# Audio-WestlakeU/FS-EEND

Measured on AMD Instinct MI355X. Metric: audio frames/sec (T=500 chunks), higher is better.
Workload: dtype bf16

## Files before the change

fs-eend_amd/build.py:

```python
import os
import subprocess
import sys
from concurrent.futures import ThreadPoolExecutor

HERE = os.path.dirname(os.path.abspath(__file__))
CSRC = os.path.join(HERE, "csrc")
SOURCES = ["gemm.hip", "ffn.hip", "ffn_stream.hip", "convert_f32.hip", "convert_rows.hip", "encin.hip", "conv_stream.hip", "proj.hip", "attn.hip", "attn_full.hip", "attn_stream.hip", "spk_stream.hip", "embloss.hip", "postproc.hip", "feature.hip", "pit.hip", "misc.hip", "retention.hip", "retention_full.hip", "ret_stream.hip", "stream.hip", "stream_multi.hip", "skinny.hip", "gemm_f32.hip", "api.hip",
           "wgrad.hip", "ffn_train_stream.hip", "proj_stream.hip", "gemm_acc_stream.hip", "attn_bwd.hip", "attn_bwd_fused.hip", "train_rows.hip", "embloss_bwd.hip", "optim.hip", "api_train.hip",
           "ls_train.hip", "retention_bwd.hip"]
LIB = os.path.join(CSRC, "libeend_hip.so")
ARCH = "gfx950"
FLAGS = ["-O3", "-std=c++17", "-fPIC", f"--offload-arch={ARCH}", "-fno-gpu-rdc"]


def _hipcc():
    for c in (os.environ.get("HIPCC"), "/opt/rocm/bin/hipcc", "hipcc"):
        if c and (os.path.isabs(c) and os.path.exists(c) or not os.path.isabs(c)):
            return c
    return "hipcc"


def _stale(target, deps):
    if not os.path.exists(target):
        return True
# ... 36 lines not shown
```

fs-eend_amd/csrc/api.hip:

```cpp
#include "../../include/eend_hip.h"
#include "kernels.h"
#include <stdlib.h>
#include <string.h>

namespace {
GemmParams base_params(const void* A, int lda, const void* W, int ldw, const float* bias, int M, int N, int K) {
    GemmParams p;
    memset(&p, 0, sizeof(p));
    p.A = A; p.lda = lda; p.W = W; p.ldw = ldw; p.bias = bias;
    p.M = M; p.N = N; p.K = K; p.ldo = N; p.Tp = 64; p.H = 4; p.dh = 64; p.C = 1;
    p.alpha = 1.0f; p.eps = 1e-5f; p.conv_cin = 64; p.conv_pad = 0; p.drop.scale = 1.0f;
#ifdef EEND_GEMM_ABLATE
    const char* d = getenv("EEND_GEMM_DBG");
    p.dbg = d ? atoi(d) : 0;
#endif
    return p;
}
}

extern "C" {

int eend_abi_version(void) { return 5; }

int eend_bn_cast_pad_f16(const float* x, const float* bn_weight, const float* bn_bias, const float* bn_mean,
// ... 240 lines not shown
    return eend_launch_conv_stream(p, (hipStream_t)stream);
}

int eend_encoder_input_ok(int Fin, int Tp, int ldw) { return eend_encin_supported(Fin, Tp, ldw); }

int eend_encoder_input_f16(const float* const* x_ptrs, const int* lens, float pad_value, const float* bn_w, const float* bn_b,
                           const float* bn_mean, const float* bn_var, float bn_eps, const void* W_f16, int ldw, const float* bias,
                           const float* gamma, const float* beta, float eps, float* out_f32, void* out_f16, int B, int T, int Tp,
                           int Fin, void* stream) {
    EncInParams p;
    memset(&p, 0, sizeof(p));
    p.x_ptrs = x_ptrs; p.lens = lens; p.pad_value = pad_value; p.bn_w = bn_w; p.bn_b = bn_b; p.bn_mean = bn_mean; p.bn_var = bn_var;
    p.bn_eps = bn_eps; p.W = W_f16; p.ldw = ldw; p.bias = bias; p.gamma = gamma; p.beta = beta; p.eps = eps; p.out32 = out_f32;
    p.out16 = out_f16; p.B = B; p.T = T; p.Tp = Tp; p.Fin = Fin;
    return eend_launch_encin(p, (hipStream_t)stream);
}

int eend_spk_stream_elems(void) { return (int)eend_spk_stream_nelems(); }

int eend_spk_stream_ok(int C, int Tp) { return eend_spk_stream_supported(C, Tp); }

int eend_spk_stream_pack_f16(const void* Wo, const void* W_in, void* stream_out, void* stream) {
    return eend_launch_spk_stream_pack(Wo, W_in, stream_out, (hipStream_t)stream);
}

int eend_attnout_spk_stream_f16(const void* A, int lda, const void* wstream, const float* bo, const void* res_f16,
                                const float* g1, const float* be1, float eps1, void* x_f16, const float* b_in, void* O_f16,
                                int B, int C, int Tp, float scale, void* stream) {
    SpkStreamParams p;
    memset(&p, 0, sizeof(p));
// ... 344 lines not shown
```

fs-eend_amd/csrc/kernels.h:

```cpp
#pragma once
#include <hip/hip_runtime.h>
#include <stdint.h>
#include "../../include/eend_hip.h"
#include "common.h"

enum GemmEpilogue {
    EPI_PLAIN_F16 = 0,
    EPI_PLAIN_RELU_F16 = 1,
    EPI_QK_HEADS = 2,
    EPI_VT_HEADS = 3,
    EPI_RES_LN = 4,
    EPI_L2NORM = 5,
    EPI_CONVERT = 6,
    EPI_RES_SCALE = 7,
    EPI_RES_SCALE_LN16 = 8,
    EPI_PLAIN_SWISH_F16 = 9,
    EPI_GLU_F16 = 10,
    EPI_QK_HEADS_F16 = 11,
    EPI_KTVT_HEADS_F16 = 12,
    EPI_PLAIN_BF16 = 13,
    EPI_MASK_BF16 = 14,
    EPI_F32_ROWMASK = 15,
    EPI_RES_LN_TRAIN = 16,
    EPI_L2NORM_TRAIN = 17,
// ... 267 lines not shown
    const float* be1;
    float eps1;
    const void* res16;
    void* x16;
    const float* res32;
    float* x32;
    const float* bin;
    void* O;
    int B, C, Tp;
    float scale;
};
long eend_spk_stream_nelems();
int eend_spk_stream_supported(int C, int Tp);
int eend_launch_spk_stream_pack(const void* Wo, const void* Win, void* out, hipStream_t stream);
int eend_launch_spk_stream(const SpkStreamParams& p, hipStream_t stream);
int eend_launch_convert_fanout_rows(const void* E, const void* W1, const float* pc, float* out32, void* out16, int B, int Tp, int C,
                                    hipStream_t stream);
struct ConvStreamParams {
    const void* X;
    const void* wstream;
    const float* bias;
    const int* ilens;
    float* out32;
    void* out16;
    float* inv_norm;
    int nseq, Tp, ktaps, pad;
};
long eend_conv_stream_nelems(int ktaps);
int eend_conv_stream_supported(int cin, int ktaps, int pad);
int eend_launch_conv_stream_pack(const void* Wr, void* out, int ktaps, hipStream_t stream);
// ... 191 lines not shown
```

fs-eend_amd/fs_model.py:

```python
import copy
import math
from typing import List, Optional, Sequence

import torch
import torch.nn as nn
from torch import Tensor

from . import ops
from .lib import EendHipError

_D_SUPPORTED = 256
_H_SUPPORTED = 4


class PositionalEncoding(nn.Module):

    def __init__(self, d_model, dropout=0.1, max_len=5000):
        super().__init__()
        self.dropout = nn.Dropout(p=dropout)
        pe = torch.zeros(max_len, d_model)
        position = torch.arange(0, max_len, dtype=torch.float).unsqueeze(1)
        div_term = torch.exp(torch.arange(0, d_model, 2).float() * (-math.log(10000.0) / d_model))
        pe[:, 0::2] = torch.sin(position * div_term)
        pe[:, 1::2] = torch.cos(position * div_term)
# ... 205 lines not shown
        dl = []
        for l in self.dec.attractor_decoder.layers:
            dl.append(dict(
                in1_w=_f16(_qscaled(l.self_attn1.in_proj_weight)), in1_b=_f32(_qscaled(l.self_attn1.in_proj_bias)),
                out1_w=_f16(l.self_attn1.out_proj.weight), out1_b=_f32(l.self_attn1.out_proj.bias),
                in2_w=_f16(l.self_attn2.in_proj_weight), in2_b=_f32(l.self_attn2.in_proj_bias),
                out2_w=_f16(l.self_attn2.out_proj.weight), out2_b=_f32(l.self_attn2.out_proj.bias),
                w1=_f16(l.linear1.weight), b1=_f32(l.linear1.bias), w2=_f16(l.linear2.weight), b2=_f32(l.linear2.bias),
                g11=_f32(l.norm11.weight), be11=_f32(l.norm11.bias), eps11=l.norm11.eps,
                g21=_f32(l.norm21.weight), be21=_f32(l.norm21.bias), eps21=l.norm21.eps,
                g22=_f32(l.norm22.weight), be22=_f32(l.norm22.bias), eps22=l.norm22.eps))
        for L in dl:
            if ops.stream_ok(L["w1"].shape[0]):
                L["ws"] = ops.ffn_stream_pack(L["out2_w"], L["w1"], L["w2"])
            L["ws1"] = ops.spk_stream_pack(L["out1_w"], L["in2_w"])
            L["in1_wp"] = ops.inproj_attn_pack(L["in1_w"])
        P["dec.layers"] = dl
        self._prep, self._prep_key = P, key
        self._pc = {}
        return P

    def _convert_const(self, C):
        if C not in self._pc:
            from . import lib as _lib
            D = self.enc.n_units if hasattr(self.enc, "n_units") else self.n_units
            dev = self.dec.convert.weight.device
            W = self.dec.convert.weight.detach().to(torch.float32).contiguous()
            b = self.dec.convert.bias.detach().to(torch.float32).contiguous()
            pe = self.dec.pos_enc.pe[0, :C].to(device=dev, dtype=torch.float32).contiguous()
            pc = torch.empty(C, D, dtype=torch.float32, device=dev)
# ... 66 lines not shown
                                       L["be2"], L["eps2"], None, ws.h16)
            else:
                ops.attnout_ffn_fused_res16(o16, L["out_w"], L["out_b"], ws.h16, L["g1"], L["be1"], L["eps1"], L["w1"], L["b1"],
                                            L["w2"], L["b2"], L["g2"], L["be2"], L["eps2"], None, ws.h16)

        emb32 = torch.empty(Me, D, dtype=torch.float32, device=dev)
        if "cnn.ws" in P:
            ops.conv1d_l2norm_stream(ws.h16, P["cnn.ws"], P["cnn.b"], il, emb32, ws.emb16, B, Tp, P["cnn.k"], P["cnn.pad"])
        else:
            ops.conv1d_l2norm(ws.h16, P["cnn.w"], P["cnn.b"], il, emb32, ws.emb16, B, Tp, D, P["cnn.k"], P["cnn.pad"])

        ops.convert_fanout(ws.emb16, P["convert.w1"], self._convert_const(C), None, ws.a16, B, Tp, C)
        o16 = ws.o16[:Md]
        for L in P["dec.layers"]:
            time_attention(ws.a16, L, "in1_w", "in1_b", B * C, self.dec.mask_delay, T)
            ops.attnout_spk_stream(o16, L["ws1"], L["out1_b"], ws.a16, L["g11"], L["be11"], L["eps11"], ws.a16, L["in2_b"], o16, B, C, Tp)
            if "ws" in L:
                ops.attnout_ffn_stream(o16, L["ws"], L["out2_b"], None, ws.a16, L["g21"], L["be21"], L["eps21"], L["b1"], L["b2"],
                                       L["g22"], L["be22"], L["eps22"], None, ws.a16)
            else:
                ops.attnout_ffn_fused_res16(o16, L["out2_w"], L["out2_b"], ws.a16, L["g21"], L["be21"], L["eps21"], L["w1"], L["b1"],
                                            L["w2"], L["b2"], L["g22"], L["be22"], L["eps22"], None, ws.a16)

        attr = torch.empty(B, T, C, D, dtype=torch.float32, device=dev)
        logits = torch.empty(B, T, C, dtype=torch.float32, device=dev)
        ops.head_l2dot(emb32, ws.a16, attr, logits, B, T, Tp, C, D)
        emb = emb32.view(B, Tp, D)
        return logits, emb, attr, T, Tp

    @torch.no_grad()
# ... 23 lines not shown
```

fs-eend_amd/lib.py:

```python
import ctypes
import os

_HERE = os.path.dirname(os.path.abspath(__file__))
LIB_PATH = os.environ.get("EEND_HIP_LIB") or os.path.join(_HERE, "csrc", "libeend_hip.so")

_vp, _i, _f = ctypes.c_void_p, ctypes.c_int, ctypes.c_float
_l = ctypes.c_long

ABI_VERSION = 5

PROTOTYPES = {
    "eend_abi_version": [],
    "eend_bn_cast_pad_f16": [_vp, _vp, _vp, _vp, _vp, _f, _vp, _i, _i, _i, _i, _i, _i, _vp],
    "eend_gather_bn_cast_pad_f16": [_vp, _vp, _f, _vp, _vp, _vp, _vp, _f, _vp, _i, _i, _i, _i, _i, _i, _vp],
    "eend_linear_f16": [_vp, _i, _vp, _i, _vp, _vp, _i, _i, _i, _i, _i, _vp],
    "eend_inproj_heads_bf16": [_vp, _i, _vp, _i, _vp, _vp, _vp, _vp, _i, _i, _i, _i, _i, _vp],
    "eend_linear_glu_f16": [_vp, _i, _vp, _i, _vp, _vp, _i, _i, _i, _i, _vp],
    "eend_linear_res_ln_f16": [_vp, _i, _vp, _i, _vp, _vp, _f, _vp, _vp, _f, _vp, _vp, _i, _i, _vp],
    "eend_linear_res16_ln_f16": [_vp, _i, _vp, _i, _vp, _vp, _f, _vp, _vp, _f, _vp, _vp, _i, _i, _vp],
    "eend_linear_res_scale_ln16_f16": [_vp, _i, _vp, _i, _vp, _vp, _f, _vp, _vp, _f, _vp, _vp, _i, _i, _vp],
    "eend_ffn_fused_f16": [_vp, _i, _vp, _vp, _vp, _vp, _vp, _f, _vp, _vp, _f, _vp, _vp, _i, _i, _i, _i, _vp],
    "eend_attnout_ffn_fused_f16": [_vp, _i, _vp, _vp, _vp, _vp, _vp, _f, _vp, _vp, _vp, _vp, _vp, _vp, _f, _vp, _vp, _vp, _vp, _i, _i, _vp],
    "eend_attnout_ffn_fused_res16_f16": [_vp, _i, _vp, _vp, _vp, _vp, _vp, _f, _vp, _vp, _vp, _vp, _vp, _vp, _f, _vp, _vp, _i, _i, _vp],
    "eend_convert_fanout_f32": [_vp, _vp, _i, _vp, _vp, _vp, _vp, _i, _i, _i, _vp],
# ... 15 lines not shown
    "eend_gemm_acc_stream_elems": [_i],
    "eend_gemm_acc_stream_ok": [_i, _i, _i],
    "eend_gemm_acc_stream_pack_bf16": [_vp, _i, _vp, _i, _vp],
    "eend_gemm_acc_stream_bf16": [_vp, _i, _vp, _vp, _i, _i, _vp],
    "eend_proj_stream_elems": [_i],
    "eend_proj_stream_pack_f16": [_vp, _vp, _i, _vp],
    "eend_proj_stream_ok": [_i, _i, _i, _i, _i, _vp],
    "eend_proj_stream_f16": [_vp, _i, _vp, _vp, _i, _i, _i, _i, _vp, _vp],
    "eend_inproj_attn_long_scratch_elems": [_i, _i, _i, _i, _vp, _vp],
    "eend_inproj_attn_causal_long_f16": [_vp, _i, _vp, _vp, _vp, _vp, _vp, _i, _i, _i, _i, _i, _i, _vp],
    "eend_spk_stream_elems": [],
    "eend_spk_stream_ok": [_i, _i],
    "eend_spk_stream_pack_f16": [_vp, _vp, _vp, _vp],
    "eend_attnout_spk_stream_f16": [_vp, _i, _vp, _vp, _vp, _vp, _vp, _f, _vp, _vp, _vp, _i, _i, _i, _f, _vp],
    "eend_attnout_spk_stream_res32_f16": [_vp, _i, _vp, _vp, _vp, _vp, _vp, _f, _vp, _vp, _vp, _i, _i, _i, _f, _vp],
    "eend_ffn_stream_max_rows": [_i],
    "eend_debug_ffn_stream_set": [_i, _l],
    "eend_attnout_ffn_stream_f16": [_vp, _i, _vp, _vp, _vp, _vp, _vp, _vp, _f, _vp, _vp, _vp, _vp, _f, _vp, _vp, _i, _i, _vp],
    "eend_emb_consistency_f32": [_vp, _vp, _vp, _f, _vp, _vp, _i, _i, _i, _i, _i, _vp],
    "eend_activity_median_u8": [_vp, _i, _i, _i, _f, _i, _vp, _vp],
    "eend_activity_segments_i32": [_vp, _i, _i, _vp, _vp, _i, _vp],
    "eend_der_counters_u64": [_vp, _i, _vp, _i, _i, _i, _i, _vp, _vp],
    "eend_stft_logmel23_f32": [_vp, _l, _l, _i, _vp, _vp, _vp, _vp],
    "eend_feature_meannorm_f32": [_vp, _vp, _i, _i, _i, _vp],
    "eend_splice_subsample_f32": [_vp, _i, _i, _i, _i, _vp, _vp],
    "eend_pit_cost_f64": [_vp, _vp, _i, _i, _i, _vp, _vp],
    "eend_pit_assign_i32": [_vp, _vp, _i, _i, _vp, _vp, _vp],
    "eend_retention_proj_f16": [_vp, _i, _vp, _i, _vp, _vp, _vp, _vp, _vp, _vp, _i, _i, _i, _i, _i, _vp],
    "eend_retention_chunk_f16": [_vp, _vp, _vp, _vp, _vp, _vp, _vp, _vp, _vp, _vp, _i, _i, _i, _i, _i, _i, _f, _i, _vp, _vp, _vp],
    "eend_retention_stream_elems": [],
# ... 137 lines not shown
```

fs-eend_amd/ops.py:

```python
import math

import torch

from . import lib as _lib

F16, BF16, F32 = torch.float16, torch.bfloat16, torch.float32


def _stream():
    return torch.cuda.current_stream().cuda_stream


def _p(t):
    return None if t is None else t.data_ptr()


def _chk(t, dtype, name):
    if t is None:
        return
    if not t.is_cuda:
        raise _lib.EendHipError(f"{name}: expected a GPU tensor (the HIP path has no CPU fallback)")
    if t.dtype != dtype:
        raise _lib.EendHipError(f"{name}: expected {dtype}, got {t.dtype}")
    if not t.is_contiguous():
# ... 352 lines not shown

def attnout_spk_stream_res32(a16, wstream, bo, res32, g1, be1, eps1, x32, b_in, out16, B, C, Tp):
    L = _lib.load()
    _chk(a16, F16, "a16"); _chk(wstream, F16, "wstream"); _chk(res32, F32, "res32"); _chk(x32, F32, "x32"); _chk(out16, F16, "out16")
    for n, t in (("bo", bo), ("g1", g1), ("be1", be1), ("b_in", b_in)):
        _chk(t, F32, n)
    M = B * C * Tp
    if a16.shape != (M, 256) or res32.shape != (M, 256) or x32.shape != (M, 256) or out16.shape != (M, 256) or b_in.numel() != 768:
        raise _lib.EendHipError("attnout_spk_stream_res32: shape mismatch")
    if wstream.numel() != L.eend_spk_stream_elems():
        raise _lib.EendHipError("attnout_spk_stream_res32: weight stream has the wrong size")
    _lib.check(L.eend_attnout_spk_stream_res32_f16(_p(a16), a16.stride(0), _p(wstream), _p(bo), _p(res32), _p(g1), _p(be1), eps1, _p(x32),
                                                   _p(b_in), _p(out16), B, C, Tp, 0.125, _stream()), "eend_attnout_spk_stream_res32_f16")


def spk_attn(qkv16, o16, B, C, Tp, H):
    L = _lib.load()
    _chk(qkv16, F16, "qkv16"); _chk(o16, F16, "o16")
    _lib.check(L.eend_spk_attn_f16(_p(qkv16), _p(o16), B, C, Tp, H, 1.0 / math.sqrt(64.0), _stream()),
               "eend_spk_attn_f16")


def emb_consistency(emb32, labels, T, lens=None, inv_count=0.0):
    L = _lib.load()
    _chk(emb32, F32, "emb32"); _chk(labels, F32, "labels"); _chk(lens, torch.int32, "lens")
    B, Tp, D = emb32.shape
    if labels.shape[0] != B or labels.shape[1] != T or Tp < T:
        raise _lib.EendHipError("emb_consistency: shape mismatch")
    nt = (T + 63) // 64
    ws = torch.empty(B * nt * nt, dtype=F32, device=emb32.device)
# ... 387 lines not shown
```

include/eend_hip.h:

```cpp
#ifndef EEND_HIP_H
#define EEND_HIP_H

#ifdef __cplusplus
extern "C" {
#endif

#define EEND_OK 0
#define EEND_EINVAL (-1)
#define EEND_ELAUNCH (-2)

#define EEND_ABI_VERSION 5
int eend_abi_version(void);

int eend_bn_cast_pad_f16(const float* x, const float* bn_weight, const float* bn_bias,
                         const float* bn_mean, const float* bn_var, float eps, void* out_f16,
                         int B, int T, int Tp, int Fin, int Fpad, int apply_bn, void* stream);

int eend_gather_bn_cast_pad_f16(const void* const* x_ptrs, const int* lens, float pad_value,
                                const float* bn_weight, const float* bn_bias, const float* bn_mean,
                                const float* bn_var, float eps, void* out_f16, int B, int T, int Tp, int Fin,
                                int Fpad, int apply_bn, void* stream);

int eend_encoder_input_ok(int Fin, int Tp, int ldw);
int eend_encoder_input_f16(const float* const* x_ptrs, const int* lens, float pad_value, const float* bn_w, const float* bn_b,
// ... 72 lines not shown
                                   float eps2, float* out_f32, void* out_f16, void* out_lo_f16, int M, int F, void* stream);
int eend_attnout_ffn_stream_f16(const void* A, int lda, const void* wstream, const float* bo, const float* res,
                                const void* res_f16, const float* g1, const float* be1, float eps1, const float* b1,
                                const float* b2, const float* g2, const float* be2, float eps2,
                                float* out_f32, void* out_f16, int M, int F, void* stream);

int eend_spk_stream_elems(void);
int eend_spk_stream_ok(int C, int Tp);
int eend_spk_stream_pack_f16(const void* Wo, const void* W_in, void* stream_out, void* stream);
int eend_attnout_spk_stream_f16(const void* A, int lda, const void* wstream, const float* bo, const void* res_f16,
                                const float* g1, const float* be1, float eps1, void* x_f16, const float* b_in, void* O_f16,
                                int B, int C, int Tp, float scale, void* stream);
int eend_attnout_spk_stream_res32_f16(const void* A, int lda, const void* wstream, const float* bo, const float* res_f32,
                                      const float* g1, const float* be1, float eps1, float* x_f32, const float* b_in, void* O_f16,
                                      int B, int C, int Tp, float scale, void* stream);


int eend_emb_consistency_f32(const float* emb, const float* labels, const int* lens, float inv_count,
                             float* partial_ws, float* out, int B, int T, int Tp, int D, int C, void* stream);


int eend_activity_median_u8(const float* pred, int ld, int T, int S, float threshold, int median,
                            unsigned char* act, void* stream);

int eend_activity_segments_i32(const unsigned char* act, int T, int S, int* changes, int* counts, int cap,
                               void* stream);

int eend_der_counters_u64(const float* pred, int ldp, const float* label, int ldl, int T, int C, int label_delay,
                          unsigned long long* counters, void* stream);

// ... 287 lines not shown
```

Before: 16.60 million.

## Fuse decoder attn-out, speaker attention and FFN into one streaming kernel

Adds a persistent streaming kernel that runs the decoder layer's time-attention output projection with residual LayerNorm, the speaker-axis attention, its output projection with LayerNorm, and the FFN with final LayerNorm in a single launch. Weights are packed into a slot stream and DMA'd into LDS through a multi-slot ring, while activations stay in registers. The model uses this path when the C/Tp configuration is supported, replacing two separate kernels and the HBM round trip of the intermediate between them. The cost is heavy register and LDS pressure at one block per CU, and the path only covers C of 3 or 6.

```diff
diff --git a/fs-eend_amd/build.py b/fs-eend_amd/build.py
--- a/fs-eend_amd/build.py
+++ b/fs-eend_amd/build.py
@@ -5,7 +5,7 @@
 
 HERE = os.path.dirname(os.path.abspath(__file__))
 CSRC = os.path.join(HERE, "csrc")
-SOURCES = ["gemm.hip", "ffn.hip", "ffn_stream.hip", "convert_f32.hip", "convert_rows.hip", "encin.hip", "conv_stream.hip", "proj.hip", "attn.hip", "attn_full.hip", "attn_stream.hip", "spk_stream.hip", "embloss.hip", "postproc.hip", "feature.hip", "pit.hip", "misc.hip", "retention.hip", "retention_full.hip", "ret_stream.hip", "stream.hip", "stream_multi.hip", "skinny.hip", "gemm_f32.hip", "api.hip",
+SOURCES = ["gemm.hip", "ffn.hip", "ffn_stream.hip", "convert_f32.hip", "convert_rows.hip", "encin.hip", "conv_stream.hip", "proj.hip", "attn.hip", "attn_full.hip", "attn_stream.hip", "spk_stream.hip", "dec_stream.hip", "embloss.hip", "postproc.hip", "feature.hip", "pit.hip", "misc.hip", "retention.hip", "retention_full.hip", "ret_stream.hip", "stream.hip", "stream_multi.hip", "skinny.hip", "gemm_f32.hip", "api.hip",
            "wgrad.hip", "ffn_train_stream.hip", "proj_stream.hip", "gemm_acc_stream.hip", "attn_bwd.hip", "attn_bwd_fused.hip", "train_rows.hip", "embloss_bwd.hip", "optim.hip", "api_train.hip",
            "ls_train.hip", "retention_bwd.hip"]
 LIB = os.path.join(CSRC, "libeend_hip.so")
diff --git a/fs-eend_amd/csrc/api.hip b/fs-eend_amd/csrc/api.hip
--- a/fs-eend_amd/csrc/api.hip
+++ b/fs-eend_amd/csrc/api.hip
@@ -278,6 +278,27 @@
     p.bn_eps = bn_eps; p.W = W_f16; p.ldw = ldw; p.bias = bias; p.gamma = gamma; p.beta = beta; p.eps = eps; p.out32 = out_f32;
     p.out16 = out_f16; p.B = B; p.T = T; p.Tp = Tp; p.Fin = Fin;
     return eend_launch_encin(p, (hipStream_t)stream);
+}
+
+int eend_dec_stream_elems(int F) { return F >= 64 && F % 64 == 0 && F <= 2048 ? (int)eend_dec_stream_nelems(F) : 0; }
+
+int eend_dec_stream_ok(int C, int Tp) { return eend_dec_stream_supported(C, Tp); }
+
+int eend_dec_stream_pack_f16(const void* Wo1, const void* W_in, const void* Wo2, const void* W1, const void* W2, void* stream_out, int F,
+                             void* stream) {
+    return eend_launch_dec_stream_pack(Wo1, W_in, Wo2, W1, W2, stream_out, F, (hipStream_t)stream);
+}
+
+int eend_attnout_spk_ffn_stream_f16(const void* A, int lda, const void* wstream, const float* bo1, const void* res_f16, const float* g11,
+                                    const float* be11, float eps11, const float* b_in, const float* bo2, const float* g21, const float* be21,
+                                    float eps21, const float* b1, const float* b2, const float* g22, const float* be22, float eps22,
+                                    void* out_f16, int B, int C, int Tp, int F, float scale, void* stream) {
+    DecStreamParams p;
+    memset(&p, 0, sizeof(p));
+    p.A = A; p.lda = lda; p.wstream = wstream; p.bo1 = bo1; p.g11 = g11; p.be11 = be11; p.eps11 = eps11; p.res16 = res_f16; p.bin = b_in;
+    p.bo2 = bo2; p.g21 = g21; p.be21 = be21; p.eps21 = eps21; p.b1 = b1; p.b2 = b2; p.g22 = g22; p.be22 = be22; p.eps22 = eps22;
+    p.out16 = out_f16; p.B = B; p.C = C; p.Tp = Tp; p.F = F; p.scale = scale;
+    return eend_launch_dec_stream(p, (hipStream_t)stream);
 }
 
 int eend_spk_stream_elems(void) { return (int)eend_spk_stream_nelems(); }
diff --git a/fs-eend_amd/csrc/dec_stream.hip b/fs-eend_amd/csrc/dec_stream.hip
--- /dev/null
+++ b/fs-eend_amd/csrc/dec_stream.hip
@@ -0,0 +1,574 @@
+#include "common.h"
+#include "kernels.h"
+#include <type_traits>
+#include <utility>
+
+namespace {
+
+template <class F, int... I>
+__device__ __forceinline__ void sfor_impl(F&& f, std::integer_sequence<int, I...>) { (f(std::integral_constant<int, I>{}), ...); }
+template <int N, class F>
+__device__ __forceinline__ void sfor(F&& f) { sfor_impl(f, std::make_integer_sequence<int, N>{}); }
+template <int V> using IC = std::integral_constant<int, V>;
+
+typedef __attribute__((address_space(3))) char lds_char;
+typedef unsigned u32x4 __attribute__((ext_vector_type(4)));
+typedef float f32x2 __attribute__((ext_vector_type(2)));
+
+constexpr int NJ = 3;
+constexpr int SLOT = 16384;
+constexpr int NSLOT = 8;
+constexpr int STAGE = NSLOT * SLOT;
+constexpr int VECS = STAGE + 4 * 2048;
+constexpr int B1L = VECS + 11 * 1024;
+constexpr int MAXF = 2048;
+constexpr int SMEM = B1L + MAXF * 4;
+constexpr int NB = 8;
+constexpr int PD = 6;
+constexpr int INFL = 4 * (NSLOT - 3);
+constexpr int NSPK = 32;
+constexpr int NHEAD = NSPK + 8;
+enum { V_BO1, V_G11, V_BE11, V_BQ, V_BV, V_BO2, V_G21, V_BE21, V_B2, V_G22, V_BE22 };
+
+__global__ void dec_stream_pack_kernel(const _Float16* __restrict__ Wo1, const _Float16* __restrict__ Win, const _Float16* __restrict__ Wo2,
+                                       const _Float16* __restrict__ W1, const _Float16* __restrict__ W2, _Float16* __restrict__ out, int F) {
+    const int U = F / 32;
+    const long total = (long)(NHEAD + 2 * U) * (SLOT / 16);
+    for (long t = (long)blockIdx.x * blockDim.x + threadIdx.x; t < total; t += (long)gridDim.x * blockDim.x) {
+        const int item = (int)(t >> 10), w = (int)(t & 1023);
+        const int pfrag = w >> 6, l = w & 63, f = l & 15, g = l >> 4;
+        const int n = (f >> 2) * 64 + pfrag * 4 + (f & 3);
+        _Float16 v[8];
+        if (item < 8) {
+            const int kc = item >> 1, sl = item & 1;
+            const _Float16* src = Wo1 + (size_t)n * 256 + kc * 64 + sl * 32 + g * 8;
+#pragma unroll
+            for (int e = 0; e < 8; ++e) v[e] = src[e];
+        } else if (item < NSPK) {
+            const int q = item - 8, h = q / 6, tt = (q % 6) >> 1, u = q & 1;
+            const int s_ = pfrag >> 1, hf = pfrag & 1;
+            const _Float16* src = Win + (size_t)(tt * 256 + h * 64 + (f >> 2) * 16 + (u * 2 + hf) * 4 + (f & 3)) * 256 + g * 64 + 8 * s_;
+#pragma unroll
+            for (int e = 0; e < 8; ++e) v[e] = src[e];
+        } else if (item < NHEAD) {
+            const int h = (item - NSPK) >> 1, u = (item - NSPK) & 1;
+            const _Float16* src = Wo2 + (size_t)n * 256 + h * 64 + g * 16 + u * 8;
+#pragma unroll
+            for (int e = 0; e < 8; ++e) v[e] = src[e];
+        } else {
+            const int q = item - NHEAD;
+            bool is_w1;
+            int k;
+            if (q == 0) { is_w1 = true; k = 0; }
+            else if (q == 2 * U - 1) { is_w1 = false; k = U - 1; }
+            else if (q & 1) { is_w1 = true; k = (q + 1) >> 1; }
+            else { is_w1 = false; k = (q >> 1) - 1; }
+            if (is_w1) {
+                const int s_ = pfrag >> 1, hf = pfrag & 1;
+                const _Float16* src = W1 + (size_t)(k * 32 + hf * 16 + f) * 256 + g * 64 + 8 * s_;
+#pragma unroll
+                for (int e = 0; e < 8; ++e) v[e] = src[e];
+            } else {
+                const _Float16* src = W2 + (size_t)n * F + k * 32 + g * 4;
+#pragma unroll
+                for (int e = 0; e < 8; ++e) v[e] = src[(e >> 2) * 16 + (e & 3)];
+            }
+        }
+        _Float16* dst = out + t * 8;
+#pragma unroll
+        for (int e = 0; e < 8; ++e) dst[e] = v[e];
+    }
+}
+
+template <int N>
+__device__ __forceinline__ float row_rot(float x) {
+    if constexpr (N == 0) return x;
+    else return __builtin_bit_cast(float, __builtin_amdgcn_update_dpp(0, __builtin_bit_cast(int, x), 0x120 + N, 0xF, 0xF, false));
+}
+
+template <int G, int CC>
+__global__ __launch_bounds__(256, 1)
+void dec_stream_kernel(const DecStreamParams p) {
+    constexpr int R = 16 / G, C = 3 * R;
+    constexpr bool FULL = CC == C;
+    static_assert(CC >= 1 && CC <= C, "slot count beyond the positions of this tiling");
+    extern __shared__ __attribute__((aligned(16))) char smem[];
+    const int TPB = p.Tp / (4 * G);
+    const int ntiles = p.B * TPB;
+    const int M = p.B * CC * p.Tp;
+    const int U = p.F >> 5;
+    const int S = NHEAD + 2 * U;
+
+    int tid = threadIdx.x;
+    asm volatile("" : "+v"(tid));
+    int lane = tid & 63;
+    const int wave = __builtin_amdgcn_readfirstlane(tid >> 6);
+    int frow = lane & 15, g = lane >> 4;
+    int fo = g * 64;
+
+    const __amdgpu_buffer_rsrc_t rs = __builtin_amdgcn_make_buffer_rsrc((void*)p.wstream, 0, S * SLOT, 0x00020000);
+    const __amdgpu_buffer_rsrc_t rsA = __builtin_amdgcn_make_buffer_rsrc((void*)p.A, 0, (M - 1) * p.lda * 2 + 512, 0x00020000);
+    const __amdgpu_buffer_rsrc_t rsR = __builtin_amdgcn_make_buffer_rsrc((void*)p.res16, 0, M * 512, 0x00020000);
+    const __amdgpu_buffer_rsrc_t rsO = __builtin_amdgcn_make_buffer_rsrc(p.out16, 0, M * 512, 0x00020000);
+    auto bload = [&](const __amdgpu_buffer_rsrc_t& r, int off) __attribute__((always_inline)) { return __builtin_amdgcn_raw_buffer_load_b128(r, off, 0, 0); };
+    int dvo = lane * 16 + wave * 4096;
+    int nxt = 0;
+    int slot = 0;
+
+    auto dma_piece = [&](int sd, auto I) __attribute__((always_inline)) {
+        constexpr int i = decltype(I)::value;
+        __builtin_amdgcn_raw_ptr_buffer_load_lds(rs, (lds_char*)(smem + sd * SLOT + wave * 4096 + i * 1024), 16, dvo,
+                                                 nxt * SLOT + i * 1024, 0, 0);
+    };
+    auto dma_advance = [&]() __attribute__((always_inline)) { nxt = nxt + 1 == S ? 0 : nxt + 1; };
+
+    sfor<NSLOT - 1>([&](auto IT) __attribute__((always_inline)) {
+        sfor<4>([&](auto I) __attribute__((always_inline)) { dma_piece(decltype(IT)::value, I); });
+        dma_advance();
+    });
+
+    float* vecs = (float*)(smem + VECS);
+    float* b1l = (float*)(smem + B1L);
+    {
+        vecs[V_BO1 * 256 + tid] = p.bo1[tid];
+        vecs[V_G11 * 256 + tid] = p.g11[tid];
+        vecs[V_BE11 * 256 + tid] = p.be11[tid];
+        vecs[V_BQ * 256 + tid] = p.bin[tid];
+        vecs[V_BV * 256 + tid] = p.bin[512 + tid];
+        vecs[V_BO2 * 256 + tid] = p.bo2[tid];
+        vecs[V_G21 * 256 + tid] = p.g21[tid];
+        vecs[V_BE21 * 256 + tid] = p.be21[tid];
+        vecs[V_B2 * 256 + tid] = p.b2[tid];
+        vecs[V_G22 * 256 + tid] = p.g22[tid];
+        vecs[V_BE22 * 256 + tid] = p.be22[tid];
+        for (int i = tid; i < p.F; i += 256) b1l[i] = p.b1[i];
+    }
+    auto vec4 = [&](int which, int i) __attribute__((always_inline)) { return *(const f32x4*)(vecs + which * 256 + fo + i * 4); };
+
+    const char* wl = smem + lane * 16;
+    f16x8 wf[NB];
+    f32x4 acc[16][NJ];
+    f32x4 qkv[12][NJ];
+    f16x8 xf[8][NJ];
+    f16x8 ob[8][NJ];
+    f32x4 h[2][NJ];
+    f16x8 hbA[NJ], hbB[NJ];
+    f32x4 bcv[2];
+    f16x8 r8[NJ][8];
+
+    auto slot_of = [&](int j, int fr) __attribute__((always_inline)) { return j * R + fr / G; };
+    auto row_tok = [&](int tile, int j, int fr) __attribute__((always_inline)) {
+        const int b = tile / TPB, tt = tile - b * TPB;
+        int c = slot_of(j, fr);
+        if constexpr (!FULL) c = c < CC ? c : CC - 1;
+        return (b * CC + c) * p.Tp + tt * (4 * G) + wave * G + (fr % G);
+    };
+    auto load_in_frags = [&](int tile, auto J) __attribute__((always_inline)) {
+        constexpr int j = decltype(J)::value;
+        const int off = row_tok(tile, j, frow) * (p.lda * 2) + g * 16;
+#pragma unroll
+        for (int s = 0; s < 8; ++s) xf[s][j] = __builtin_bit_cast(f16x8, bload(rsA, off + s * 64));
+    };
+    auto load_res16 = [&](int tile, auto J) __attribute__((always_inline)) {
+        constexpr int j = decltype(J)::value;
+        const int off = row_tok(tile, j, frow) * 512 + fo * 2;
+#pragma unroll
+        for (int e = 0; e < 8; ++e) r8[j][e] = __builtin_bit_cast(f16x8, bload(rsR, off + e * 16));
+    };
+
+    __builtin_amdgcn_s_waitcnt(0x0070 | ((4 * (NSLOT - 2)) & 15) | (((4 * (NSLOT - 2)) >> 4) << 14));
+    __builtin_amdgcn_s_barrier();
+    sfor<NJ>([&](auto J) __attribute__((always_inline)) { load_in_frags(blockIdx.x, J); });
+
+    auto act_cvt = [&](float v) __attribute__((always_inline)) -> _Float16 {
+        return (_Float16)__builtin_amdgcn_fmed3f(v, 0.f, 65504.f);
+    };
+    auto conv_part = [&](auto PART, f16x8 (&hbo)[NJ]) __attribute__((always_inline)) {
+        constexpr int hf = decltype(PART)::value / NJ, j = decltype(PART)::value % NJ;
+#pragma unroll
+        for (int r = 0; r < 4; ++r) hbo[j][hf * 4 + r] = act_cvt(h[hf][j][r]);
+    };
+
+    auto step = [&](auto KIND, auto SRCc, auto CONVc, auto COLDc, auto PFNc, auto VWXc, int k, f16x8 (&hb)[NJ],
+                    f16x8 (&hbo)[NJ]) __attribute__((always_inline)) {
+        constexpr int kind = decltype(KIND)::value, src = decltype(SRCc)::value, vw = INFL + decltype(VWXc)::value;
+        constexpr bool conv = decltype(CONVc)::value, cold = decltype(COLDc)::value, pfn = decltype(PFNc)::value;
+        static_assert(vw <= 63, "vmcnt is a 6-bit field");
+        __builtin_amdgcn_s_waitcnt(0x0F70 | (vw & 15) | ((vw >> 4) << 14));
+        __builtin_amdgcn_s_barrier();
+        const char* wc = wl + slot * SLOT;
+        const char* wn = wl + ((slot + 1) & (NSLOT - 1)) * SLOT;
+        const int sd = (slot + NSLOT - 1) & (NSLOT - 1);
+        if constexpr (cold) {
+            sfor<PD>([&](auto Q) __attribute__((always_inline)) {
+                wf[decltype(Q)::value % NB] = *(const f16x8*)(wc + decltype(Q)::value * 1024);
+            });
+        }
+        if constexpr (kind == 3) {
+            bcv[0] = *(const f32x4*)(b1l + k * 32 + g * 4);
+            bcv[1] = *(const f32x4*)(b1l + k * 32 + 16 + g * 4);
+        }
+        sfor<8>([&](auto P2) __attribute__((always_inline)) {
+            sfor<2>([&](auto PH) __attribute__((always_inline)) {
+                constexpr int pi = decltype(P2)::value * 2 + decltype(PH)::value;
+                const f16x8 w = wf[pi % NB];
+                if constexpr (kind == 0) {
+#pragma unroll
+                    for (int j = 0; j < NJ; ++j) acc[pi][j] = __builtin_amdgcn_mfma_f32_16x16x32_f16(w, xf[src][j], acc[pi][j], 0, 0, 0);
+                } else if constexpr (kind == 1) {
+                    constexpr int s_ = pi >> 1, hf = pi & 1, idx = src * 2 + hf;
+#pragma unroll
+                    for (int j = 0; j < NJ; ++j)
+                        qkv[idx][j] = __builtin_amdgcn_mfma_f32_16x16x32_f16(w, xf[s_][j], s_ == 0 ? f32x4{0.f, 0.f, 0.f, 0.f} : qkv[idx][j], 0, 0, 0);
+                } else if constexpr (kind == 2) {
+#pragma unroll
+                    for (int j = 0; j < NJ; ++j) acc[pi][j] = __builtin_amdgcn_mfma_f32_16x16x32_f16(w, ob[src][j], acc[pi][j], 0, 0, 0);
+                } else if constexpr (kind == 3) {
+                    constexpr int s_ = pi >> 1, hf = pi & 1;
+#pragma unroll
+                    for (int j = 0; j < NJ; ++j) {
+                        if constexpr (s_ == 0)
+                            asm volatile("v_mfma_f32_16x16x32_f16 %0, %1, %2, %3" : "=&v"(h[hf][j]) : "v"(w), "v"(xf[s_][j]), "v"(bcv[hf]));
+                        else
+                            asm volatile("v_mfma_f32_16x16x32_f16 %0, %1, %2, %0" : "+v"(h[hf][j]) : "v"(w), "v"(xf[s_][j]));
+                    }
+                } else {
+#pragma unroll
+                    for (int j = 0; j < NJ; ++j) acc[pi][j] = __builtin_amdgcn_mfma_f32_16x16x32_f16(w, hb[j], acc[pi][j], 0, 0, 0);
+                }
+                if constexpr (pi + PD < 16) wf[(pi + PD) % NB] = *(const f16x8*)(wc + (pi + PD) * 1024);
+                else if constexpr (pfn) wf[(pi + PD) % NB] = *(const f16x8*)(wn + (pi + PD - 16) * 1024);
+                if constexpr (pi < 4) dma_piece(sd, IC<pi>{});
+                if constexpr (kind == 4 && conv && pi >= 2 && pi < 2 + 4 * NJ && !(pi & 1)) conv_part(IC<(pi - 2) / 2>{}, hbo);
+            });
+            __builtin_amdgcn_sched_barrier(0);
+        });
+        dma_advance();
+        slot = (slot + 1) & (NSLOT - 1);
+    };
+    auto pin_acc = [&]() __attribute__((always_inline)) {
+#pragma unroll
+        for (int i = 0; i < 16; ++i)
+#pragma unroll
+            for (int j = 0; j < NJ; ++j) asm volatile("" : "+a"(acc[i][j]));
+    };
+
+    for (int tile = blockIdx.x; tile < ntiles; tile += gridDim.x) {
+        auto relaunder = [&]() __attribute__((always_inline)) {
+            asm volatile("v_mbcnt_lo_u32_b32 %0, -1, 0\n\tv_mbcnt_hi_u32_b32 %0, -1, %0" : "=v"(lane));
+            frow = lane & 15; g = lane >> 4; fo = g * 64;
+            dvo = lane * 16 + wave * 4096;
+            wl = smem + lane * 16;
+        };
+        relaunder();
+        const int ntile = tile + (int)gridDim.x;
+        using T = std::true_type;
+        using Fa = std::false_type;
+
+#pragma unroll
+        for (int i = 0; i < 16; ++i) {
+            const f32x4 b4 = vec4(V_BO1, i);
+#pragma unroll
+            for (int j = 0; j < NJ; ++j) acc[i][j] = b4;
+        }
+        pin_acc();
+        step(IC<0>{}, IC<0>{}, Fa{}, T{}, T{}, IC<24>{}, 0, hbA, hbB);
+        step(IC<0>{}, IC<1>{}, Fa{}, Fa{}, T{}, IC<24>{}, 0, hbA, hbB);
+        step(IC<0>{}, IC<2>{}, Fa{}, Fa{}, T{}, IC<24>{}, 0, hbA, hbB);
+        step(IC<0>{}, IC<3>{}, Fa{}, Fa{}, T{}, IC<24>{}, 0, hbA, hbB);
+        step(IC<0>{}, IC<4>{}, Fa{}, Fa{}, T{}, IC<24>{}, 0, hbA, hbB);
+        step(IC<0>{}, IC<5>{}, Fa{}, Fa{}, T{}, IC<24>{}, 0, hbA, hbB);
+        step(IC<0>{}, IC<6>{}, Fa{}, Fa{}, T{}, IC<0>{}, 0, hbA, hbB);
+        load_res16(tile, IC<0>{});
+        step(IC<0>{}, IC<7>{}, Fa{}, Fa{}, Fa{}, IC<8>{}, 0, hbA, hbB);
+        pin_acc();
+        relaunder();
+        sfor<NJ>([&](auto J) __attribute__((always_inline)) {
+            constexpr int j = decltype(J)::value;
+            auto resv = [&](int i, int q) __attribute__((always_inline)) { return (float)r8[j][i >> 1][(i & 1) * 4 + q]; };
+            f32x2 sm = f32x2{0.f, 0.f}, sq2 = f32x2{0.f, 0.f};
+#pragma unroll
+            for (int i = 0; i < 16; ++i) {
+                const f32x4 a4 = acc[i][j];
+                const f32x2 x0 = f32x2{a4[0] + resv(i, 0), a4[1] + resv(i, 1)};
+                const f32x2 x1 = f32x2{a4[2] + resv(i, 2), a4[3] + resv(i, 3)};
+                sm += x0 + x1;
+                sq2 = x1 * x1 + (x0 * x0 + sq2);
+            }
+            const float sum = wave_g_allreduce_add(sm[0] + sm[1]);
+            const float sqs = wave_g_allreduce_add(sq2[0] + sq2[1]);
+            const float mean = sum * (1.0f / 256);
+            const float var = __builtin_fmaxf(sqs * (1.0f / 256) - mean * mean, 0.f);
+            const float rstd = 1.0f / __builtin_sqrtf(var + p.eps11);
+            __builtin_amdgcn_sched_barrier(0);
+            if constexpr (j + 1 < NJ) load_res16(tile, IC<j + 1>{});
+#pragma unroll
+            for (int i = 0; i < 16; ++i) {
+                const f32x4 gg = vec4(V_G11, i) * rstd, bb = vec4(V_BE11, i) - vec4(V_G11, i) * (rstd * mean);
+                const f32x4 a4 = acc[i][j];
+#pragma unroll
+                for (int q = 0; q < 4; ++q) xf[i >> 1][j][(i & 1) * 4 + q] = (_Float16)__builtin_fmaf(a4[q] + resv(i, q), gg[q], bb[q]);
+                if ((i & 3) == 3) __builtin_amdgcn_sched_barrier(0);
+            }
+#pragma unroll
+            for (int s = 0; s < 8; ++s) asm volatile("" : "+v"(xf[s][j]));
+            __builtin_amdgcn_sched_barrier(0);
+        });
+
+        float kbias[FULL ? 1 : C];
+        if constexpr (!FULL) {
+            sfor<NJ>([&](auto J2) __attribute__((always_inline)) {
+                constexpr int j2 = decltype(J2)::value;
+                const float own = slot_of(j2, frow) < CC ? 0.f : -1e30f;
+                sfor<R>([&](auto D) __attribute__((always_inline)) { kbias[j2 * R + decltype(D)::value] = row_rot<decltype(D)::value * G>(own); });
+            });
+        }
+        sfor<4>([&](auto HEAD) __attribute__((always_inline)) {
+            constexpr int head = decltype(HEAD)::value;
+            constexpr int yng = head == 0 ? 16 : 0;
+            step(IC<1>{}, IC<0>{}, Fa{}, T{}, T{}, IC<yng>{}, 0, hbA, hbB);
+            step(IC<1>{}, IC<1>{}, Fa{}, Fa{}, T{}, IC<yng>{}, 0, hbA, hbB);
+            step(IC<1>{}, IC<2>{}, Fa{}, Fa{}, T{}, IC<yng>{}, 0, hbA, hbB);
+            step(IC<1>{}, IC<3>{}, Fa{}, Fa{}, T{}, IC<yng>{}, 0, hbA, hbB);
+            step(IC<1>{}, IC<4>{}, Fa{}, Fa{}, T{}, IC<yng>{}, 0, hbA, hbB);
+            step(IC<1>{}, IC<5>{}, Fa{}, Fa{}, Fa{}, IC<yng>{}, 0, hbA, hbB);
+
+            const float* bq = vecs + V_BQ * 256 + head * 64 + g * 16;
+            const float* bv = vecs + V_BV * 256 + head * 64 + g * 16;
+            f32x4 bnext = *(const f32x4*)bq;
+            f32x2 s2[NJ][C];
+#pragma unroll
+            for (int a = 0; a < NJ; ++a)
+#pragma unroll
+                for (int c = 0; c < C; ++c) s2[a][c] = f32x2{0.f, 0.f};
+            sfor<4>([&](auto FF) __attribute__((always_inline)) {
+                constexpr int ff = decltype(FF)::value;
+                const f32x4 b4 = bnext;
+                bnext = ff < 3 ? *(const f32x4*)(bq + (ff + 1) * 4) : *(const f32x4*)bv;
+                f32x2 q[NJ][2];
+#pragma unroll
+                for (int j = 0; j < NJ; ++j) {
+                    const f32x4 t = (qkv[ff][j] + b4) * p.scale;
+                    q[j][0] = f32x2{t[0], t[1]}; q[j][1] = f32x2{t[2], t[3]};
+                }
+                sfor<NJ>([&](auto J2) __attribute__((always_inline)) {
+                    constexpr int j2 = decltype(J2)::value;
+                    const f32x4 k = qkv[4 + ff][j2];
+                    sfor<R>([&](auto D) __attribute__((always_inline)) {
+                        constexpr int d = decltype(D)::value;
+                        const f32x2 k0 = f32x2{row_rot<d * G>(k[0]), row_rot<d * G>(k[1])};
+                        const f32x2 k1 = f32x2{row_rot<d * G>(k[2]), row_rot<d * G>(k[3])};
+#pragma unroll
+                        for (int j1 = 0; j1 < NJ; ++j1) s2[j1][j2 * R + d] = q[j1][1] * k1 + (q[j1][0] * k0 + s2[j1][j2 * R + d]);
+                    });
+                });
+            });
+            float s[NJ][C];
+#pragma unroll
+            for (int a = 0; a < NJ; ++a) {
+                float mx = -INFINITY, den = 0.f;
+#pragma unroll
+                for (int c = 0; c < C; ++c) {
+                    s[a][c] = s2[a][c][0] + s2[a][c][1];
+                    if constexpr (!FULL) s[a][c] += kbias[c];
+                    s[a][c] = wave_g_allreduce_add(s[a][c]);
+                    mx = __builtin_fmaxf(mx, s[a][c]);
+                }
+#pragma unroll
+                for (int c = 0; c < C; ++c) { s[a][c] = __expf(s[a][c] - mx); den += s[a][c]; }
+                const float inv = __builtin_amdgcn_rcpf(den);
+#pragma unroll
+                for (int c = 0; c < C; ++c) s[a][c] *= inv;
+            }
+            sfor<4>([&](auto FF) __attribute__((always_inline)) {
+                constexpr int ff = decltype(FF)::value;
+                const f32x4 b4 = bnext;
+                if constexpr (ff < 3) bnext = *(const f32x4*)(bv + (ff + 1) * 4);
+                f32x2 o[NJ][2];
+#pragma unroll
+                for (int j = 0; j < NJ; ++j) { o[j][0] = f32x2{b4[0], b4[1]}; o[j][1] = f32x2{b4[2], b4[3]}; }
+                sfor<NJ>([&](auto J2) __attribute__((always_inline)) {
+                    constexpr int j2 = decltype(J2)::value;
+                    const f32x4 vv = qkv[8 + ff][j2];
+                    sfor<R>([&](auto D) __attribute__((always_inline)) {
+                        constexpr int d = decltype(D)::value;
+                        const f32x2 v0 = f32x2{row_rot<d * G>(vv[0]), row_rot<d * G>(vv[1])};
+                        const f32x2 v1 = f32x2{row_rot<d * G>(vv[2]), row_rot<d * G>(vv[3])};
+#pragma unroll
+                        for (int j1 = 0; j1 < NJ; ++j1) {
+                            const f32x2 pw = f32x2{s[j1][j2 * R + d], s[j1][j2 * R + d]};
+                            o[j1][0] = pw * v0 + o[j1][0];
+                            o[j1][1] = pw * v1 + o[j1][1];
+                        }
+                    });
+                });
+                constexpr int ui = head * 2 + (ff >> 1);
+#pragma unroll
+                for (int j = 0; j < NJ; ++j) {
+                    ob[ui][j][(ff & 1) * 4 + 0] = to_f16_sat(o[j][0][0]); ob[ui][j][(ff & 1) * 4 + 1] = to_f16_sat(o[j][0][1]);
+                    ob[ui][j][(ff & 1) * 4 + 2] = to_f16_sat(o[j][1][0]); ob[ui][j][(ff & 1) * 4 + 3] = to_f16_sat(o[j][1][1]);
+                }
+            });
+            __builtin_amdgcn_sched_barrier(0);
+        });
+
+        relaunder();
+#pragma unroll
+        for (int i = 0; i < 16; ++i) {
+            const f32x4 b4 = vec4(V_BO2, i);
+#pragma unroll
+            for (int j = 0; j < NJ; ++j) acc[i][j] = b4;
+        }
+        pin_acc();
+        step(IC<2>{}, IC<0>{}, Fa{}, T{}, T{}, IC<0>{}, 0, hbA, hbB);
+        step(IC<2>{}, IC<1>{}, Fa{}, Fa{}, T{}, IC<0>{}, 0, hbA, hbB);
+        step(IC<2>{}, IC<2>{}, Fa{}, Fa{}, T{}, IC<0>{}, 0, hbA, hbB);
+        step(IC<2>{}, IC<3>{}, Fa{}, Fa{}, T{}, IC<0>{}, 0, hbA, hbB);
+        step(IC<2>{}, IC<4>{}, Fa{}, Fa{}, T{}, IC<0>{}, 0, hbA, hbB);
+        step(IC<2>{}, IC<5>{}, Fa{}, Fa{}, T{}, IC<0>{}, 0, hbA, hbB);
+        step(IC<2>{}, IC<6>{}, Fa{}, Fa{}, T{}, IC<0>{}, 0, hbA, hbB);
+        step(IC<2>{}, IC<7>{}, Fa{}, Fa{}, Fa{}, IC<0>{}, 0, hbA, hbB);
+        pin_acc();
+        relaunder();
+        sfor<NJ>([&](auto J) __attribute__((always_inline)) {
+            constexpr int j = decltype(J)::value;
+            auto xval = [&](int i, int q) __attribute__((always_inline)) { return acc[i][j][q] + (float)xf[i >> 1][j][(i & 1) * 4 + q]; };
+            f32x2 sm = f32x2{0.f, 0.f}, sq2 = f32x2{0.f, 0.f};
+#pragma unroll
+            for (int i = 0; i < 16; ++i) {
+                const f32x2 x0 = f32x2{xval(i, 0), xval(i, 1)}, x1 = f32x2{xval(i, 2), xval(i, 3)};
+                sm += x0 + x1;
+                sq2 = x1 * x1 + (x0 * x0 + sq2);
+            }
+            const float sum = wave_g_allreduce_add(sm[0] + sm[1]);
+            const float sqs = wave_g_allreduce_add(sq2[0] + sq2[1]);
+            const float mean = sum * (1.0f / 256);
+            const float rstd = 1.0f / __builtin_sqrtf(__builtin_fmaxf(sqs * (1.0f / 256) - mean * mean, 0.f) + p.eps21);
+            __builtin_amdgcn_sched_barrier(0);
+#pragma unroll
+            for (int i = 0; i < 16; ++i) {
+                const f32x4 g4 = vec4(V_G21, i), gg = g4 * rstd, bb = vec4(V_BE21, i) - g4 * (rstd * mean), b2 = vec4(V_B2, i);
+                f32x4 xo;
+#pragma unroll
+                for (int q = 0; q < 4; ++q) {
+                    const float x = __builtin_fmaf(xval(i, q), gg[q], bb[q]);
+                    xf[i >> 1][j][(i & 1) * 4 + q] = (_Float16)x;
+                    xo[q] = x + b2[q];
+                }
+                acc[i][j] = xo;
+                if ((i & 3) == 3) __builtin_amdgcn_sched_barrier(0);
+            }
+        });
+
+        relaunder();
+        pin_acc();
+        step(IC<3>{}, IC<0>{}, Fa{}, T{}, Fa{}, IC<0>{}, 0, hbA, hbB);
+        asm volatile("s_nop 15\n\ts_nop 7" ::: "memory");
+        sfor<2 * NJ>([&](auto Q) __attribute__((always_inline)) { conv_part(Q, hbA); });
+        step(IC<3>{}, IC<0>{}, Fa{}, T{}, T{}, IC<0>{}, 1, hbA, hbB);
+        for (int k = 2; k < U; k += 2) {
+            relaunder();
+            step(IC<4>{}, IC<0>{}, T{}, Fa{}, T{}, IC<0>{}, 0, hbA, hbB);
+            step(IC<3>{}, IC<0>{}, Fa{}, Fa{}, T{}, IC<0>{}, k, hbA, hbB);
+            step(IC<4>{}, IC<0>{}, T{}, Fa{}, T{}, IC<0>{}, 0, hbB, hbA);
+            step(IC<3>{}, IC<0>{}, Fa{}, Fa{}, T{}, IC<0>{}, k + 1, hbA, hbB);
+        }
+        sfor<NJ>([&](auto J) __attribute__((always_inline)) { load_in_frags(ntile, J); });
+        step(IC<4>{}, IC<0>{}, T{}, Fa{}, T{}, IC<8 * NJ>{}, 0, hbA, hbB);
+        step(IC<4>{}, IC<0>{}, Fa{}, Fa{}, Fa{}, IC<8 * NJ>{}, 0, hbB, hbA);
+        pin_acc();
+
+        relaunder();
+        char* st = smem + STAGE + wave * 2048;
+        sfor<NJ>([&](auto J) __attribute__((always_inline)) {
+            constexpr int j = decltype(J)::value;
+            f32x2 sm = f32x2{0.f, 0.f}, sq2 = f32x2{0.f, 0.f};
+#pragma unroll
+            for (int i = 0; i < 16; ++i) {
+                const f32x4 a4 = acc[i][j];
+                const f32x2 x0 = f32x2{a4[0], a4[1]}, x1 = f32x2{a4[2], a4[3]};
+                sm += x0 + x1;
+                sq2 = x1 * x1 + (x0 * x0 + sq2);
+            }
+            const float sum = wave_g_allreduce_add(sm[0] + sm[1]);
+            const float sqs = wave_g_allreduce_add(sq2[0] + sq2[1]);
+            const float mean = sum * (1.0f / 256);
+            const float rstd = 1.0f / __builtin_sqrtf(__builtin_fmaxf(sqs * (1.0f / 256) - mean * mean, 0.f) + p.eps22);
+            __builtin_amdgcn_sched_barrier(0);
+            f16x8 o[8];
+#pragma unroll
+            for (int i = 0; i < 16; ++i) {
+                const f32x4 g4 = vec4(V_G22, i), gg = g4 * rstd, bb = vec4(V_BE22, i) - g4 * (rstd * mean);
+                const f32x4 a4 = acc[i][j];
+#pragma unroll
+                for (int q = 0; q < 4; ++q) o[i >> 1][(i & 1) * 4 + q] = (_Float16)__builtin_fmaf(a4[q], gg[q], bb[q]);
+                if ((i & 3) == 3) __builtin_amdgcn_sched_barrier(0);
+            }
+#pragma unroll
+            for (int qr = 0; qr < 4; ++qr) {
+                if ((frow >> 2) == qr) {
+#pragma unroll
+                    for (int e = 0; e < 8; ++e) *(f16x8*)(st + (frow & 3) * 512 + (((g * 8 + e) ^ (frow & 3)) << 4)) = o[e];
+                }
+                wave_lds_sync();
+#pragma unroll
+                for (int q2 = 0; q2 < 2; ++q2) {
+                    const int rr = 2 * q2 + (lane >> 5), cc = lane & 31, fr = qr * 4 + rr;
+                    const f16x8 v = *(const f16x8*)(st + rr * 512 + ((cc ^ rr) << 4));
+                    const int off = (FULL || slot_of(j, fr) < CC) ? row_tok(tile, j, fr) * 512 + cc * 16 : 0x7FFFFFF0;
+                    __builtin_amdgcn_raw_buffer_store_b128(__builtin_bit_cast(u32x4, v), rsO, off, 0, 0);
+                }
+                wave_lds_sync();
+            }
+            __builtin_amdgcn_sched_barrier(0);
+        });
+    }
+    asm volatile("s_waitcnt vmcnt(0)" ::: "memory");
+}
+
+template <int G, int CC>
+int launch(const DecStreamParams& p, hipStream_t stream) {
+    static EendOncePerDevice attr_once;
+    auto kern = dec_stream_kernel<G, CC>;
+    if (!eend_set_dynamic_lds(attr_once, (const void*)kern, SMEM)) return EEND_ELAUNCH;
+    const int ncu = eend_cu_count();
+    const int ntiles = p.B * (p.Tp / (4 * G));
+    hipLaunchKernelGGL(kern, dim3(ntiles < ncu ? ntiles : ncu), dim3(256), SMEM, stream, p);
+    return hipGetLastError() == hipSuccess ? EEND_OK : EEND_ELAUNCH;
+}
+
+constexpr int frames_per_wave(int C) { return C <= 3 ? 16 : C <= 6 ? 8 : 4; }
+
+}
+
+long eend_dec_stream_nelems(int F) { return (long)(NHEAD + 2 * (F / 32)) * (SLOT / 2); }
+
+int eend_dec_stream_supported(int C, int Tp) {
+    if (C != 3 && C != 6) return 0;
+    return Tp > 0 && Tp % (4 * frames_per_wave(C)) == 0;
+}
+
+int eend_launch_dec_stream_pack(const void* Wo1, const void* Win, const void* Wo2, const void* W1, const void* W2, void* out, int F,
+                                hipStream_t stream) {
+    if (!Wo1 || !Win || !Wo2 || !W1 || !W2 || !out || F < 64 || F > MAXF || (F % 64) != 0) return EEND_EINVAL;
+    const long total = eend_dec_stream_nelems(F) / 8;
+    const int blocks = (int)((total + 255) / 256);
+    hipLaunchKernelGGL(dec_stream_pack_kernel, dim3(blocks < 4096 ? blocks : 4096), dim3(256), 0, stream, (const _Float16*)Wo1,
+                       (const _Float16*)Win, (const _Float16*)Wo2, (const _Float16*)W1, (const _Float16*)W2, (_Float16*)out, F);
+    return hipGetLastError() == hipSuccess ? EEND_OK : EEND_ELAUNCH;
+}
+
+int eend_launch_dec_stream(const DecStreamParams& p, hipStream_t stream) {
+    if (!p.A || !p.wstream || !p.bo1 || !p.g11 || !p.be11 || !p.res16 || !p.bin || !p.bo2 || !p.g21 || !p.be21 || !p.b1 || !p.b2 ||
+        !p.g22 || !p.be22 || !p.out16 || p.B <= 0 || p.lda < 256 || (p.lda & 7) || !eend_dec_stream_supported(p.C, p.Tp) || p.F < 64 ||
+        p.F > MAXF || (p.F % 64) != 0)
+        return EEND_EINVAL;
+    const long rows = (long)p.B * p.C * p.Tp + 65536;
+    if (rows * p.lda * 2 >= (1L << 31) || rows * 512 >= (1L << 31)) return EEND_EINVAL;
+    switch (p.C) {
+#define DEC_CASE(n) case n: return launch<frames_per_wave(n), n>(p, stream);
+        DEC_CASE(3) DEC_CASE(6)
+#undef DEC_CASE
+        default: return EEND_EINVAL;
+    }
+}
diff --git a/fs-eend_amd/csrc/kernels.h b/fs-eend_amd/csrc/kernels.h
--- a/fs-eend_amd/csrc/kernels.h
+++ b/fs-eend_amd/csrc/kernels.h
@@ -305,6 +305,34 @@
 int eend_spk_stream_supported(int C, int Tp);
 int eend_launch_spk_stream_pack(const void* Wo, const void* Win, void* out, hipStream_t stream);
 int eend_launch_spk_stream(const SpkStreamParams& p, hipStream_t stream);
+struct DecStreamParams {
+    const void* A;
+    int lda;
+    const void* wstream;
+    const float* bo1;
+    const float* g11;
+    const float* be11;
+    float eps11;
+    const void* res16;
+    const float* bin;
+    const float* bo2;
+    const float* g21;
+    const float* be21;
+    float eps21;
+    const float* b1;
+    const float* b2;
+    const float* g22;
+    const float* be22;
+    float eps22;
+    void* out16;
+    int B, C, Tp, F;
+    float scale;
+};
+long eend_dec_stream_nelems(int F);
+int eend_dec_stream_supported(int C, int Tp);
+int eend_launch_dec_stream_pack(const void* Wo1, const void* Win, const void* Wo2, const void* W1, const void* W2, void* out, int F,
+                                hipStream_t stream);
+int eend_launch_dec_stream(const DecStreamParams& p, hipStream_t stream);
 int eend_launch_convert_fanout_rows(const void* E, const void* W1, const float* pc, float* out32, void* out16, int B, int Tp, int C,
                                     hipStream_t stream);
 struct ConvStreamParams {
diff --git a/fs-eend_amd/fs_model.py b/fs-eend_amd/fs_model.py
--- a/fs-eend_amd/fs_model.py
+++ b/fs-eend_amd/fs_model.py
@@ -243,6 +243,8 @@
             if ops.stream_ok(L["w1"].shape[0]):
                 L["ws"] = ops.ffn_stream_pack(L["out2_w"], L["w1"], L["w2"])
             L["ws1"] = ops.spk_stream_pack(L["out1_w"], L["in2_w"])
+            if ops.stream_ok(L["w1"].shape[0]):
+                L["wsd"] = ops.dec_stream_pack(L["out1_w"], L["in2_w"], L["out2_w"], L["w1"], L["w2"])
             L["in1_wp"] = ops.inproj_attn_pack(L["in1_w"])
         P["dec.layers"] = dl
         self._prep, self._prep_key = P, key
@@ -339,6 +341,10 @@
         o16 = ws.o16[:Md]
         for L in P["dec.layers"]:
             time_attention(ws.a16, L, "in1_w", "in1_b", B * C, self.dec.mask_delay, T)
+            if "wsd" in L and ops.dec_stream_ok(C, Tp):
+                ops.attnout_spk_ffn_stream(o16, L["wsd"], L["out1_b"], ws.a16, L["g11"], L["be11"], L["eps11"], L["in2_b"], L["out2_b"],
+                                           L["g21"], L["be21"], L["eps21"], L["b1"], L["b2"], L["g22"], L["be22"], L["eps22"], ws.a16, B, C, Tp)
+                continue
             ops.attnout_spk_stream(o16, L["ws1"], L["out1_b"], ws.a16, L["g11"], L["be11"], L["eps11"], ws.a16, L["in2_b"], o16, B, C, Tp)
             if "ws" in L:
                 ops.attnout_ffn_stream(o16, L["ws"], L["out2_b"], None, ws.a16, L["g21"], L["be21"], L["eps21"], L["b1"], L["b2"],
diff --git a/fs-eend_amd/lib.py b/fs-eend_amd/lib.py
--- a/fs-eend_amd/lib.py
+++ b/fs-eend_amd/lib.py
@@ -53,6 +53,11 @@
     "eend_spk_stream_pack_f16": [_vp, _vp, _vp, _vp],
     "eend_attnout_spk_stream_f16": [_vp, _i, _vp, _vp, _vp, _vp, _vp, _f, _vp, _vp, _vp, _i, _i, _i, _f, _vp],
     "eend_attnout_spk_stream_res32_f16": [_vp, _i, _vp, _vp, _vp, _vp, _vp, _f, _vp, _vp, _vp, _i, _i, _i, _f, _vp],
+    "eend_dec_stream_elems": [_i],
+    "eend_dec_stream_ok": [_i, _i],
+    "eend_dec_stream_pack_f16": [_vp, _vp, _vp, _vp, _vp, _vp, _i, _vp],
+    "eend_attnout_spk_ffn_stream_f16": [_vp, _i, _vp, _vp, _vp, _vp, _vp, _f, _vp, _vp, _vp, _vp, _f, _vp, _vp, _vp, _vp, _f, _vp, _i, _i, _i,
+                                        _i, _f, _vp],
     "eend_ffn_stream_max_rows": [_i],
     "eend_debug_ffn_stream_set": [_i, _l],
     "eend_attnout_ffn_stream_f16": [_vp, _i, _vp, _vp, _vp, _vp, _vp, _vp, _f, _vp, _vp, _vp, _vp, _f, _vp, _vp, _i, _i, _vp],
diff --git a/fs-eend_amd/ops.py b/fs-eend_amd/ops.py
--- a/fs-eend_amd/ops.py
+++ b/fs-eend_amd/ops.py
@@ -390,6 +390,43 @@
                                                    _p(b_in), _p(out16), B, C, Tp, 0.125, _stream()), "eend_attnout_spk_stream_res32_f16")
 
 
+def dec_stream_pack(wo1, win, wo2, w1, w2):
+    L = _lib.load()
+    for n, t in (("wo1", wo1), ("win", win), ("wo2", wo2), ("w1", w1), ("w2", w2)):
+        _chk(t, F16, n)
+    Fh = w1.shape[0]
+    n = L.eend_dec_stream_elems(Fh)
+    if (wo1.shape != (256, 256) or win.shape != (768, 256) or wo2.shape != (256, 256) or w1.shape[1] != 256 or w2.shape != (256, Fh)
+            or n <= 0 or not all(t.is_contiguous() for t in (wo1, win, wo2, w1, w2))):
+        raise _lib.EendHipError("dec_stream_pack: expected contiguous Wo1 / Wo2 [256][256], W_in [768][256], W1 [F][256], W2 [256][F], "
+                                "F a multiple of 64 up to 2048")
+    out = torch.empty(n, dtype=F16, device=wo1.device)
+    _lib.check(L.eend_dec_stream_pack_f16(_p(wo1), _p(win), _p(wo2), _p(w1), _p(w2), _p(out), Fh, _stream()), "eend_dec_stream_pack_f16")
+    return out
+
+
+def dec_stream_ok(C, Tp):
+    return bool(_lib.load().eend_dec_stream_ok(int(C), int(Tp)))
+
+
+def attnout_spk_ffn_stream(a16, wstream, bo1, res16, g11, be11, eps11, b_in, bo2, g21, be21, eps21, b1, b2, g22, be22, eps22, out16,
+                           B, C, Tp):
+    L = _lib.load()
+    _chk(a16, F16, "a16"); _chk(wstream, F16, "wstream"); _chk(res16, F16, "res16"); _chk(out16, F16, "out16")
+    for n, t in (("bo1", bo1), ("g11", g11), ("be11", be11), ("b_in", b_in), ("bo2", bo2), ("g21", g21), ("be21", be21), ("b1", b1),
+                 ("b2", b2), ("g22", g22), ("be22", be22)):
+        _chk(t, F32, n)
+    M = B * C * Tp
+    Fh = b1.numel()
+    if a16.shape != (M, 256) or res16.shape != (M, 256) or out16.shape != (M, 256) or b_in.numel() != 768:
+        raise _lib.EendHipError("attnout_spk_ffn_stream: shape mismatch")
+    if wstream.numel() != L.eend_dec_stream_elems(Fh):
+        raise _lib.EendHipError("attnout_spk_ffn_stream: weight stream has the wrong size")
+    _lib.check(L.eend_attnout_spk_ffn_stream_f16(_p(a16), a16.stride(0), _p(wstream), _p(bo1), _p(res16), _p(g11), _p(be11), eps11,
+                                                 _p(b_in), _p(bo2), _p(g21), _p(be21), eps21, _p(b1), _p(b2), _p(g22), _p(be22), eps22,
+                                                 _p(out16), B, C, Tp, Fh, 0.125, _stream()), "eend_attnout_spk_ffn_stream_f16")
+
+
 def spk_attn(qkv16, o16, B, C, Tp, H):
     L = _lib.load()
     _chk(qkv16, F16, "qkv16"); _chk(o16, F16, "o16")
diff --git a/include/eend_hip.h b/include/eend_hip.h
--- a/include/eend_hip.h
+++ b/include/eend_hip.h
@@ -110,6 +110,14 @@
 int eend_attnout_spk_stream_res32_f16(const void* A, int lda, const void* wstream, const float* bo, const float* res_f32,
                                       const float* g1, const float* be1, float eps1, float* x_f32, const float* b_in, void* O_f16,
                                       int B, int C, int Tp, float scale, void* stream);
+int eend_dec_stream_elems(int F);
+int eend_dec_stream_ok(int C, int Tp);
+int eend_dec_stream_pack_f16(const void* Wo1, const void* W_in, const void* Wo2, const void* W1, const void* W2, void* stream_out, int F,
+                             void* stream);
+int eend_attnout_spk_ffn_stream_f16(const void* A, int lda, const void* wstream, const float* bo1, const void* res_f16, const float* g11,
+                                    const float* be11, float eps11, const float* b_in, const float* bo2, const float* g21, const float* be21,
+                                    float eps21, const float* b1, const float* b2, const float* g22, const float* be22, float eps22,
+                                    void* out_f16, int B, int C, int Tp, int F, float scale, void* stream);
 
 
 int eend_emb_consistency_f32(const float* emb, const float* labels, const int* lens, float inv_count,
```

After: 17.01 million, median of 6. 2.5% higher.
